# ubc-vision/UniT

Hardware: AMD Instinct MI355X
Metric: images/sec (fwd+bwd+SGD) R101-C4 VOC 600x1000 bs=2/GPU (higher is better)
Workload: dtype bf16; 1 GPU; UniT base-training step S1 (TrainerNoMeta.run_step): ResNet-101-C4, VOC split1 K=20, 2 supervised + 2 weak 3x600x1000 images per GPU, 512 RoIs/image, two Res5 heads, RPN 12000->2000, all 8 losses, SGD momentum; images_per_gpu=2, global_batch=2, parallelism=dp1

## Files before the change

### unit_amd/csrc/conv_igemm256.h

```cpp
#pragma once
#include "common.h"

#include "conv_epilogue.h"

struct Conv256Args {
  const void* x; const void* w; void* y;
  const float* bias; const void* residual; const void* mask_ref;
  int N, H, W, C;
  int K, R, S, stride, pad;
  int OH, OW;
  int ldy, oy_mul, OHf, OWf;
  int relu;
  int Kgemm, M;
  int tiles_m, tiles_n;
  unsigned x_bytes, w_bytes;
  EpiExtra ex;
  int ex_on;
  const void* x2; unsigned x2_bytes; int cb_split, ratio2;
  int pm_ncls;
  PmClass pm_cls[9];
  unsigned magic_ow, magic_oh;
  ConvSecond second;
  SplitK sk;
  int mask_pitch;
// ... 10 lines not shown
};
template <> struct O4<bf16_t> {
  static __device__ __forceinline__ void load(const bf16_t* p, float (&v)[4]) {
    bf16x4 a = *reinterpret_cast<const bf16x4*>(p);
#pragma unroll
    for (int i = 0; i < 4; ++i) v[i] = (float)a[i];
  }
  static __device__ __forceinline__ void store(bf16_t* p, const float (&v)[4]) {
    bf16x4 a;
#pragma unroll
    for (int i = 0; i < 4; ++i) a[i] = (bf16_t)v[i];
    *reinterpret_cast<bf16x4*>(p) = a;
  }
};

int unit_conv256_p8_launch(Conv256Args& a, int out_dtype, bool reads_in_mfma, bool rows224, hipStream_t st);
int unit_conv256_p8m_launch(Conv256Args& a, int out_dtype, hipStream_t st);
```

### unit_amd/csrc/conv_igemm256.hip

```cpp
#include "conv_igemm256.h"
#include "conv_igemm128.h"
#include "conv_pair.h"
#include "conv_epilogue.h"

#ifndef UNIT_DBG256
#define UNIT_DBG256 0
#endif

template <typename TO, bool PP, int FB>
__global__ void __launch_bounds__(512, 2) conv_igemm256_kernel(Conv256Args p) {
  constexpr int BM = 32 * FB, BMR = 256, BN = 256, BK = 64;
  constexpr int BUF = (BMR + BN) * 128;
  extern __shared__ __attribute__((aligned(16))) char smem[];

  int nwg = p.tiles_m * p.tiles_n;
  int bid = blockIdx.x;
  {
    int q = nwg / 8, r = nwg % 8, xcd = bid % 8, loc = bid / 8;
    bid = (xcd < r ? xcd * (q + 1) : r * (q + 1) + (xcd - r) * q) + loc;
  }
  int tile_n = bid % p.tiles_n, tile_m = bid / p.tiles_n;
  int m0 = tile_m * BM, n0 = tile_n * BN;

  const bf16_t* __restrict__ X = (const bf16_t*)p.x;
// ... 556 lines not shown
  a.sk = SplitK{0, 0, 0, 0}; a.mask_pitch = 0; a.second.on = 0;
  a.x = x; a.w = w; a.y = y; a.bias = bias; a.residual = residual; a.mask_ref = mask_ref;
  a.N = N; a.H = H; a.W = W; a.C = C; a.K = K; a.R = R; a.S = S; a.stride = stride; a.pad = pad;
  a.OH = OH; a.OW = OW; a.ldy = ldy; a.oy_mul = oy_mul; a.OHf = OHf; a.OWf = OWf; a.relu = relu;
  a.Kgemm = R * S * C; a.M = N * OH * OW;
  size_t xb = (size_t)N * H * W * C * 2, wb = (size_t)K * R * S * C * 2;
  UNIT_CHECK_ARG(xb < 0xFFFFFFF0ull && wb < 0xFFFFFFF0ull, "conv_big: operand larger than 4 GiB");
  a.x_bytes = (unsigned)xb; a.w_bytes = (unsigned)wb;
  a.ex = EpiExtra{nullptr, nullptr, nullptr, 0}; a.ex_on = 0;
  a.x2 = nullptr; a.x2_bytes = 0; a.cb_split = 0; a.ratio2 = 1; a.pm_ncls = 0;
  set_div_magics(a);
  { int rc = unit_fill_second(a.second, second, R, S, stride, pad, oy_mul, (size_t)C * 2); if (rc != UNIT_OK) return rc; }
  if (K == 0 || (a.M == 0 && !a.second.on)) return UNIT_OK;
  hipStream_t st = (hipStream_t)stream;
  if (variant == 0) variant = 8;
  if (a.second.on) {
    UNIT_CHECK_ARG(out_dtype == UNIT_BF16 && (ldy & 7) == 0 && (variant == 8 || variant == 12), "conv_big: pair launches: bf16 output, ldy % 8 == 0, variant 0 / 8 / 12");
    return unit_conv256_p8_launch(a, out_dtype, true, false, st);
  }
  auto fewer_with_224 = [&] {
    long n_tiles = cdiv(K, 256);
    long c256 = (long)cdiv((long)cdiv(a.M, 256) * n_tiles, 256) * 256, c224 = (long)cdiv((long)cdiv(a.M, 224) * n_tiles, 256) * 224;
    return c224 < c256;
  };
  if (variant == 6) {
    bool halo_ok = out_dtype == UNIT_BF16 && (ldy & 7) == 0 && R == 3 && S == 3 && stride == 1 && pad == 1 && H == 7 && W == 7 &&
                   OH == 7 && OW == 7;
    if (!halo_ok) { unit_set_error("conv_big: variant 6 needs a bf16-out 3x3 s1 p1 conv on 7x7 maps"); return UNIT_ERR_UNSUPPORTED; }
    return launch256_halo7(a, st);
  }
  if (variant == 11) return unit_conv256_p8m_launch(a, out_dtype, st);
  if (variant == 12) return unit_conv256_p8_launch(a, out_dtype, true, false, st);
  if (variant >= 7 && variant <= 10) {
    bool r224 = variant == 9 || (variant == 10 && fewer_with_224());
    if (variant == 8 && out_dtype == UNIT_BF16 && (ldy & 7) == 0 && R == 3 && S == 3 && stride == 1 &&
        pad == 1 && OH == H && OW == W && oy_mul == 1 && OHf == OH && OWf == OW && H * W <= 4096 && (size_t)N * H * W * ldy * 2 < 0xFFFFFFF0ull)
      build_position_classes(a);
    return unit_conv256_p8_launch(a, out_dtype, variant >= 8, r224, st);
  }
  bool rows224 = variant == 3 || (variant == 5 && fewer_with_224());
  if (out_dtype == UNIT_BF16) {
    if (variant == 2) return launch256_k32<bf16_t>(a, st);
    if (variant == 1) return launch256<bf16_t, true, 8>(a, st);
    return rows224 ? launch256<bf16_t, false, 7>(a, st) : launch256<bf16_t, false, 8>(a, st);
  }
  if (out_dtype == UNIT_F32) {
    if (variant == 2) return launch256_k32<float>(a, st);
    if (variant == 1) return launch256<float, true, 8>(a, st);
    return rows224 ? launch256<float, false, 7>(a, st) : launch256<float, false, 8>(a, st);
  }
  unit_set_error("conv_big: unsupported out dtype");
  return UNIT_ERR_UNSUPPORTED;
}
// ... 74 lines not shown
                                     second, stream, 3);
    case 4: return unit_conv_x3_impl(x, w, y, bias, residual, mask_ref, mask_c, N, H, W, C, K, R, S, stride, pad, OH, OW, ldy, oy_mul, OHf, OWf, relu, tile,
                                     second, stream, 2);
  }
  unit_set_error("conv_pair: kernel 0 (generic), 1 (mid), 2 (big), 3 (bf16x3), 4 (bf16x3, two segments)");
  return UNIT_ERR_ARG;
}


extern "C" size_t unit_conv_pool_partial_floats(int M, int ldy) { return (size_t)cdiv(M, 128) * 4 * (size_t)ldy; }

extern "C" int unit_conv2d_fwd_big_ex(const void* x, const void* w, void* y, const float* bias, const void* residual,
                                      const unsigned char* mask_bits, unsigned char* relu_bits, float* pool_partial, int pool_rows,
                                      int N, int H, int W, int C, int K, int R, int S, int pad, int ldy, int relu, const void* x2, int C2,
                                      int variant, void* stream) {
  UNIT_CHECK_ARG(variant == 0 || variant == 8 || variant == 11, "conv_big_ex: variant 0 (default), 8 (16x16x32 MFMA) or 11 (32x32x16 MFMA)");
  UNIT_CHECK_ARG(x2 == nullptr || (R == 1 && S == 1 && pad == 0 && C2 > 0 && C2 % C == 0 && ((uintptr_t)x2 % 16 == 0)),
                 "conv_big_ex: a second input needs a 1x1 conv and C2 a multiple of C");
  UNIT_CHECK_ARG(C % 64 == 0 && (x2 == nullptr || C2 % 64 == 0), "conv_big_ex: C must be a multiple of 64");
  UNIT_CHECK_ARG(ldy % 8 == 0 && ldy >= K, "conv_big_ex: ldy must be a multiple of 8 and >= K");
  UNIT_CHECK_ARG(y != nullptr || pool_partial != nullptr, "conv_big_ex: no output requested");
  UNIT_CHECK_ARG((mask_bits == nullptr && relu_bits == nullptr) || ldy % 64 == 0, "conv_big_ex: bit masks need ldy % 64 == 0");
  UNIT_CHECK_ARG(pool_partial == nullptr || pool_rows >= 44, "conv_big_ex: a 128-row wave tile must span at most 4 pooling segments");
  UNIT_CHECK_ARG(((uintptr_t)x % 16 == 0) && ((uintptr_t)w % 16 == 0) && ((uintptr_t)y % 16 == 0), "conv_big_ex: 16B alignment");
  int OH = H + 2 * pad - R + 1, OW = W + 2 * pad - S + 1;
  UNIT_CHECK_ARG(OH > 0 && OW > 0, "conv_big_ex: empty output");
  Conv256Args a;
  a.sk = SplitK{0, 0, 0, 0}; a.mask_pitch = 0; a.second.on = 0;
  a.x = x; a.w = w; a.y = y; a.bias = bias; a.residual = residual; a.mask_ref = nullptr;
  const int Ct = C + (x2 ? C2 : 0);
  a.N = N; a.H = H; a.W = W; a.C = Ct; a.K = K; a.R = R; a.S = S; a.stride = 1; a.pad = pad;
  a.OH = OH; a.OW = OW; a.ldy = ldy; a.oy_mul = 1; a.OHf = OH; a.OWf = OW; a.relu = relu;
  a.Kgemm = R * S * Ct; a.M = N * OH * OW;
  size_t xb = (size_t)N * H * W * C * 2, wb = (size_t)K * R * S * Ct * 2, x2b = x2 ? (size_t)N * H * W * C2 * 2 : 0;
  UNIT_CHECK_ARG(xb < 0xFFFFFFF0ull && wb < 0xFFFFFFF0ull && x2b < 0xFFFFFFF0ull, "conv_big_ex: operand larger than 4 GiB");
  a.x_bytes = (unsigned)xb; a.w_bytes = (unsigned)wb;
  a.x2 = x2; a.x2_bytes = (unsigned)x2b; a.cb_split = C / 64; a.ratio2 = x2 ? C2 / C : 1; a.pm_ncls = 0;
  set_div_magics(a);
  a.ex = EpiExtra{relu_bits, mask_bits, pool_partial, pool_rows}; a.ex_on = 1;
  if (a.M == 0 || K == 0) return UNIT_OK;
  if (variant == 11) return unit_conv256_p8m_launch(a, UNIT_BF16, (hipStream_t)stream);
  return unit_conv256_p8_launch(a, UNIT_BF16, true, false, (hipStream_t)stream);
}

template <typename T>
__global__ void pool_finish_kernel(const float* __restrict__ part, int R, int rows, int ldy, int K, T* __restrict__ out, int ldo) {
  int r = blockIdx.x;
  int w0 = (r * rows) / 128, w1 = (r * rows + rows - 1) / 128;
  float inv = (float)rows;
  int seg0 = r - (w0 * 128) / rows, seg1 = r - (w1 * 128) / rows;
  const float* p0 = part + ((size_t)w0 * 4 + seg0) * ldy;
  const float* p1 = part + ((size_t)w1 * 4 + seg1) * ldy;
  if ((K & 7) == 0 && (ldy & 3) == 0) {
    for (int n = threadIdx.x * 8; n < K; n += blockDim.x * 8) {
      f32x4 a0 = *reinterpret_cast<const f32x4*>(p0 + n), a1 = *reinterpret_cast<const f32x4*>(p0 + n + 4);
      f32x4 b0 = {0.f, 0.f, 0.f, 0.f}, b1 = {0.f, 0.f, 0.f, 0.f};
      if (w1 != w0) { b0 = *reinterpret_cast<const f32x4*>(p1 + n); b1 = *reinterpret_cast<const f32x4*>(p1 + n + 4); }
// ... 74 lines not shown
```

### unit_amd/csrc/conv_igemm256p8.hip

```cpp
#include "conv_igemm256.h"
#include "conv_epilogue.h"

#ifndef UNIT_DBGP8
#define UNIT_DBGP8 0
#endif

#ifdef UNIT_EPI_STAMP
__device__ unsigned long long g_stamp[32 * 16];
extern "C" int unit_debug_read_stamps(unsigned long long* host_out) {
  return (int)hipMemcpyFromSymbol(host_out, HIP_SYMBOL(g_stamp), sizeof(unsigned long long) * 32 * 16, 0, hipMemcpyDeviceToHost);
}
#define P8_STAMP(i) do { if (stamp) stamp[(i)] = __builtin_amdgcn_s_memtime(); } while (0)
#else
#define P8_STAMP(i) do { } while (0)
#endif

#define MFMA_BF16(A, B, C) __builtin_amdgcn_mfma_f32_16x16x32_bf16(__builtin_bit_cast(bf16x8, A), __builtin_bit_cast(bf16x8, B), C, 0, 0, 0)

template <typename TO, bool RM, int B1, bool X3 = false, bool PAIR = false, bool PERS = false>
__global__ void __launch_bounds__(512, 2) conv_igemm256_p8_kernel(Conv256Args p) {
  static_assert(RM || B1 == 4, "224-row tiles: RM schedule only");
  static_assert(!PAIR || (RM && B1 == 4), "pair launches: 256-row RM schedule");
  static_assert(!X3 || (RM && sizeof(TO) == 2), "bf16x3 operands: RM schedule, split bf16 output");
  static_assert(!PERS || (RM && !PAIR && sizeof(TO) == 2), "persistent tiles: RM schedule, bf16 rows through the LDS epilogue, one problem");
  constexpr int FBT = 4 + B1;
  constexpr int BM = 32 * FBT, BN = 256, BK = 64;
  constexpr int HALF = 128 * 128;
  constexpr int SX0 = 0, SW0 = HALF, SW1 = 2 * HALF, SX1 = 3 * HALF, BUF = 4 * HALF;
  constexpr int EPI_OFF = PERS ? BUF + SX1 : 0;
  extern __shared__ __attribute__((aligned(16))) char smem[];

  int bid = blockIdx.x;
  if constexpr (PAIR) {
    if (p.second.on && bid >= p.second.tiles0) { bid -= p.second.tiles0; pair_swap_common(p); p.magic_ow = p.second.magic_ow; p.magic_oh = p.second.magic_oh; }
  }
// ... 23 lines not shown
    int q = nwg / 8, r = nwg % 8, xcd = v % 8, loc = v / 8;
    int t = (xcd < r ? xcd * (q + 1) : r * (q + 1) + (xcd - r) * q) + loc;
    tile_n = t % p.tiles_n; tile_m = t / p.tiles_n;
  };
  if (!pm) map_tile(bid);
  int m0 = tile_m * BM, n0 = tile_n * BN;

  const bf16_t* __restrict__ X = (const bf16_t*)p.x;
  const bf16_t* __restrict__ Wt = (const bf16_t*)p.w;
  __amdgpu_buffer_rsrc_t rsX = __builtin_amdgcn_make_buffer_rsrc(const_cast<bf16_t*>(X), 0, (int)p.x_bytes, 0x00020000);
  __amdgpu_buffer_rsrc_t rsW = __builtin_amdgcn_make_buffer_rsrc(const_cast<bf16_t*>(Wt), 0, (int)p.w_bytes, 0x00020000);
  const bool dual = !X3 && p.x2 != nullptr;
  const int Cx = X3 ? p.sk.x_pitch : (dual ? p.cb_split * 64 : p.C);
  __amdgpu_buffer_rsrc_t rsX2 = __builtin_amdgcn_make_buffer_rsrc(const_cast<bf16_t*>((const bf16_t*)(dual ? p.x2 : p.x)), 0, (int)(dual ? p.x2_bytes : p.x_bytes), 0x00020000);
  constexpr unsigned OOB = 0xFFFFFFF0u;

  int tid = threadIdx.x, lane = tid & 63;
  int wid = __builtin_amdgcn_readfirstlane(tid >> 6);
  int wm = wid >> 2, wn = wid & 3;
  const int grp = wm;
  unsigned long long* stamp = nullptr;
#ifdef UNIT_EPI_STAMP
  if (tid == 0 && blockIdx.x % 97 == 0 && blockIdx.x / 97 < 32) {
    stamp = g_stamp + (blockIdx.x / 97) * 16;
    stamp[14] = blockIdx.x; stamp[15] = __builtin_amdgcn_s_memrealtime();
  }
#endif
  P8_STAMP(0);
  int lrow = lane >> 3, lc = lane & 7;

  const bool pointwise = PERS || (p.R == 1 && p.S == 1 && p.stride == 1 && p.pad == 0);
  int x_ih0[4], x_iw0[4]; unsigned x_off0[4], w_off[4];
  const unsigned sw16 = (unsigned)((lc ^ ((((wid * 8 + lrow) >> 1)) & 7)) * 16);
  auto setup_tile = [&](int lrow, int lc) {
#pragma unroll
  for (int q = 0; q < 2; ++q)
#pragma unroll
    for (int j = 0; j < 2; ++j) {
      int R = (j * 8 + wid) * 8 + lrow;
      int sw = lc ^ ((R >> 1) & 7);
      int m = m0 + (R >> 6) * (FBT * 16) + q * 64 + (R & 63);
      bool ok = m < p.M && (q == 0 || (R & 63) < B1 * 16);
      int mm = ok ? m : 0;
      int ow, oh, n;
      if (pm) {
        ok = pmr.map(m - m0, n, oh, ow);
        if (!ok) n = 0;
      } else if (pointwise) {
        n = 0; oh = 0; ow = 0;
      } else {
        unsigned t = fast_div((unsigned)mm, (unsigned)p.OW, p.magic_ow);
        ow = mm - (int)t * p.OW;
        n = (int)fast_div(t, (unsigned)p.OH, p.magic_oh);
        oh = (int)t - n * p.OH;
      }
      int ih0 = oh * p.stride - p.pad, iw0 = ow * p.stride - p.pad;
      x_off0[q * 2 + j] = pointwise ? ((unsigned)mm * (unsigned)Cx + (unsigned)(sw * 8)) * 2u
                                    : ((unsigned)n * (unsigned)(p.H * p.W * Cx) + (unsigned)((ih0 * p.W + iw0) * Cx + sw * 8)) * 2u;
      if constexpr (PERS) {
        if (!ok) x_off0[q * 2 + j] = OOB;
      } else {
        x_ih0[q * 2 + j] = ok ? ih0 : -(1 << 20);
        x_iw0[q * 2 + j] = iw0;
      }
      int nn = n0 + (R >> 5) * 64 + q * 32 + (R & 31);
      w_off[q * 2 + j] = nn < p.K ? ((unsigned)nn * (unsigned)p.Kgemm + (unsigned)sw * 8u) * 2u : OOB;
    }
  };
  setup_tile(lrow, lc);

  int r_lo = 0, r_hi = p.R - 1, s_lo = 0, s_hi = p.S - 1;
  if (pm) {
    r_lo = max(0, p.pad - pmr.oh0); r_hi = min(p.R - 1, p.H - 1 + p.pad - (pmr.oh0 + pm_nh - 1));
    s_lo = max(0, p.pad - pmr.ow0); s_hi = min(p.S - 1, p.W - 1 + p.pad - (pmr.ow0 + pmr.cw - 1));
  }
  int st_cb = 0, st_r = r_lo, st_s = s_lo;
  int st_sg = 0, st_cbr = 0;
  unsigned st_kx = (unsigned)((st_r * p.W + st_s) * Cx) * 2u, st_kw = (unsigned)((st_r * p.S + st_s) * p.C) * 2u;
  if constexpr (X3) st_kx += (unsigned)((p.sk.seg_lo & 1) * p.sk.cr) * 2u;
  auto st_reset = [&]() {
    st_cb = 0; st_r = r_lo; st_s = s_lo; st_sg = 0; st_cbr = 0;
// ... 36 lines not shown
      unsigned o = w_off[q * 2 + j];
      __builtin_amdgcn_raw_ptr_buffer_load_lds(rsW, (lds_void*)(base + (j * 8 + wid) * 1024), 16, o == OOB ? OOB : o + st_kw, 0, 0, 0);
    }
  };

  f32x4 acc[4][FBT];
  auto zero_acc = [&]() {
#pragma unroll
    for (int a = 0; a < 4; ++a)
#pragma unroll
      for (int b = 0; b < FBT; ++b) acc[a][b] = f32x4{0.f, 0.f, 0.f, 0.f};
  };
  zero_acc();

  const int nk = pm ? (p.C / BK) * (r_hi - r_lo + 1) * (s_hi - s_lo + 1) : p.Kgemm / BK;
  const int frow = lane & 15, fq = lane >> 4;
  const int fsw = (fq ^ ((frow >> 1) & 7)) << 4;
  const int offx = (wm * 64 + frow) * 128 + fsw;
  const int offw = (wn * 32 + frow) * 128 + fsw;

  i32x4 fx[4][2], fw0[2][2], fw1[2][2];
  auto read_x = [&](const char* half) {
#pragma unroll
    for (int b = 0; b < 4; ++b) {
      fx[b][0] = *reinterpret_cast<const i32x4*>(half + b * 2048 + offx);
      fx[b][1] = *reinterpret_cast<const i32x4*>(half + b * 2048 + (offx ^ 64));
    }
  };
  auto read_w = [&](const char* half, i32x4 (&fw)[2][2]) {
#pragma unroll
// ... 47 lines not shown
        }
      }
      if constexpr (RM && B1 == 4) {
        if (pm) {
          epilogue_rows_bf16_dispatch<4, FBT, false, true, false, EPI_BIAS | EPI_RELU | EPI_Y, EPI_MK | EPI_Y, EPI_Y>(
              acc, smem + EPI_OFF + wid * EpiCfg<4>::BYTES, nullptr, wm * (FBT * 16), n0e + wn * 64, p, lane, &pmr);
          return;
        }
      }
      epilogue_rows_bf16_dispatch<4, FBT, false, false, false, EPI_FULL | EPI_BIAS | EPI_RELU | EPI_Y, EPI_FULL | EPI_BIAS | EPI_Y, EPI_FULL | EPI_Y,
                                  EPI_FULL | EPI_MK | EPI_Y, EPI_FULL | EPI_RES | EPI_MK | EPI_Y, EPI_BIAS | EPI_RELU | EPI_Y, EPI_MK | EPI_Y>(
          acc, smem + EPI_OFF + wid * EpiCfg<4>::BYTES, nullptr, m0e + wm * (FBT * 16), n0e + wn * 64, p, lane, nullptr, stamp ? stamp + 4 : nullptr);
    }
  };

  if constexpr (RM) {
    constexpr int RD_PER = 1;
    i32x4 fxb[B1][2];
    auto read_xb = [&](const char* half) {
#pragma unroll
      for (int b = 0; b < B1; ++b) {
        fxb[b][0] = *reinterpret_cast<const i32x4*>(half + b * 2048 + offx);
        fxb[b][1] = *reinterpret_cast<const i32x4*>(half + b * 2048 + (offx ^ 64));
      }
    };
#define P8_MM(QX, QW, FW, FX, NB, NR, PER, READS)                                        \
    do {                                                                                 \
      __builtin_amdgcn_s_setprio(1);                                                     \
      READS;                                                                             \
      _Pragma("unroll") for (int ks = 0; ks < 2; ++ks)                                   \
        _Pragma("unroll") for (int a = 0; a < 2; ++a)                                    \
// ... 11 lines not shown
      stage_x(0, 0); stage_w(0, 0); stage_w(1, 0); stage_x(1, 0);
      st_advance();
      if (nk > 1) { stage_x(0, 1); stage_w(0, 1); stage_w(1, 1); }
    };
    prologue_stage();
    if (nk > 1) asm volatile("s_waitcnt vmcnt(6)" ::: "memory");
    else asm volatile("s_waitcnt vmcnt(0)" ::: "memory");
    int pers_v = blockIdx.x;
    while (true) {
    P8_BAR();
    P8_STAMP(1);
    read_w(smem + SW0, fw0);
    read_x(smem + SX0);
    asm volatile("s_waitcnt lgkmcnt(0)" ::: "memory");
    if (grp == 1) P8_BAR();
    for (int t = 0; t < nk; ++t) {
      const int d = t & 1;
      const char* buf = smem + d * BUF;
      const char* bnx = smem + (d ^ 1) * BUF;
      const bool n1 = t + 1 < nk, n2 = t + 2 < nk;
      if (n1) stage_x(1, d ^ 1);
      st_advance();
      P8_BAR();
      P8_MM(0, 0, fw0, fx, 4, 4, 1, read_w(buf + SW1, fw1));
      P8_BAR();
      if (n2) stage_x(0, d);
      P8_BAR();
      P8_MM(0, 1, fw1, fx, 4, 2 * B1, RD_PER, read_xb(buf + SX1));
      P8_BAR();
      if (n2) {
        stage_w(0, d);
        asm volatile("s_waitcnt vmcnt(4)" ::: "memory");
      } else {
        asm volatile("s_waitcnt vmcnt(0)" ::: "memory");
      }
      P8_BAR();
      P8_MM(1, 0, fw0, fxb, B1, 0, 1, (void)0);
      P8_BAR();
      if (n2) stage_w(1, d);
      P8_BAR();
      P8_MM(1, 1, fw1, fxb, B1, 12, RD_PER, read_w(bnx + SW0, fw0); read_x(bnx + SX0));
      P8_BAR();
    }
    if (grp == 0) P8_BAR();
    if constexpr (!PERS) break;
    else {
      P8_STAMP(2);
      __syncthreads();
      P8_STAMP(3);
      const int m0e = m0, n0e = n0, nv = pers_v + (int)gridDim.x;
      const bool more = nv < nwg;
      const bool early = more && !(p.ex_on && p.ex.pool_partial != nullptr);
      int lane_o = lane;
      asm volatile("" : "+v"(lane_o));
      auto next_tile = [&]() { map_tile(nv); m0 = tile_m * BM; n0 = tile_n * BN; setup_tile(lane_o >> 3, lane_o & 7); st_reset(); prologue_stage(); };
      if (early) next_tile();
      lds_epilogue(m0e, n0e, lane_o);
      if (!more) return;
      if (!early) { __syncthreads(); next_tile(); }
// ... 56 lines not shown
    P8_MFMA(1, 1, fw1);
    P8_BAR();
  }
  if (grp == 0) P8_BAR();
  }
#undef P8_MFMA
#undef P8_FMA
#undef P8_RD
#undef P8_BAR

  if constexpr (sizeof(TO) == 2) {
    if ((p.ldy & 7) == 0) {
      P8_STAMP(2);
      __syncthreads();
      P8_STAMP(3);
      lds_epilogue(m0, n0, lane);
      P8_STAMP(13);
      return;
    }
  }
  TO* __restrict__ Y = (TO*)p.y;
  const TO* __restrict__ Rz = (const TO*)p.residual;
  const TO* __restrict__ Mk = (const TO*)p.mask_ref;
  bool plain = (p.oy_mul == 1 && p.OHf == p.OH && p.OWf == p.OW);
#pragma unroll
  for (int b = 0; b < FBT; ++b) {
    int m = m0 + wm * (FBT * 16) + b * 16 + frow;
    if (m >= p.M) continue;
    long off;
    if (plain) off = (long)m * p.ldy;
// ... 17 lines not shown
      }
      if (p.relu) {
#pragma unroll
        for (int j = 0; j < 4; ++j) v[j] = fmaxf(v[j], 0.f);
      }
      if (Mk) {
        float mm[4]; O4<TO>::load(Mk + off + n, mm);
#pragma unroll
        for (int j = 0; j < 4; ++j) v[j] = mm[j] > 0.f ? v[j] : 0.f;
      }
      O4<TO>::store(Y + off + n, v);
    }
  }
}

template <typename TO, bool RM, int B1, bool X3 = false>
static int launch256_p8(Conv256Args& a, hipStream_t st) {
  if (a.second.on) {
    if constexpr (RM && B1 == 4 && sizeof(TO) == 2) {
      a.pm_ncls = 0;
      a.tiles_m = cdiv(a.M, 256); a.tiles_n = cdiv(a.K, 256);
      a.second.tiles_m = cdiv(a.second.M, 256);
      a.second.tiles0 = a.tiles_m * a.tiles_n;
      size_t lds2 = 8 * 128 * 128;
      static bool attr2 = false;
      if (!attr2) {
        (void)hipFuncSetAttribute((const void*)conv_igemm256_p8_kernel<TO, RM, B1, X3, true>, hipFuncAttributeMaxDynamicSharedMemorySize, (int)lds2);
        attr2 = true;
      }
      conv_igemm256_p8_kernel<TO, RM, B1, X3, true><<<(a.tiles_m + a.second.tiles_m) * a.tiles_n, 512, lds2, st>>>(a);
      UNIT_LAUNCH_CHECK();
      return UNIT_OK;
    } else {
      unit_set_error("conv_big: pair launches need the 256-row RM schedule with bf16 output");
      return UNIT_ERR_UNSUPPORTED;
    }
  }
  if (a.pm_ncls == 0) a.tiles_m = cdiv(a.M, 32 * (4 + B1));
  a.tiles_n = cdiv(a.K, 256);
  int grid = a.tiles_m * a.tiles_n;
  if (a.pm_ncls > 0) {
    if (!RM || B1 != 4) { unit_set_error("conv_big: position-class tiles need the 256-row RM schedule"); return UNIT_ERR_UNSUPPORTED; }
    int most = 0;
    for (int x = 0; x < 8; ++x) {
      int cnt = 0;
// ... 1 lines not shown
        int tc = (c + 1 < a.pm_ncls ? a.pm_cls[c + 1].tile0 : a.tiles_m) - a.pm_cls[c].tile0;
        cnt += ((x + 1) * tc + 7) / 8 - (x * tc + 7) / 8;
      }
      most = cnt > most ? cnt : most;
    }
    grid = most * 8 * a.tiles_n;
  }
  size_t lds = 8 * 128 * 128;
  if constexpr (RM && B1 == 4 && sizeof(TO) == 2) {
    const char* pe = getenv("UNIT_P8_PERSIST");
    const int pers = pe ? atoi(pe) : 1;
    if (pers && a.pm_ncls == 0 && (a.ldy & 7) == 0 && grid > 256 && a.R == 1 && a.S == 1 && a.stride == 1 && a.pad == 0) {
      const size_t lds_p = 7 * 128 * 128 + 8 * EpiCfg<4>::BYTES;
      static bool attr_p = false;
      if (!attr_p) {
        (void)hipFuncSetAttribute((const void*)conv_igemm256_p8_kernel<TO, RM, B1, X3, false, true>, hipFuncAttributeMaxDynamicSharedMemorySize, (int)lds_p);
        attr_p = true;
      }
      static int ncu = 0;
      if (ncu == 0) {
        int dev = 0, n = 0;
        if (hipGetDevice(&dev) != hipSuccess || hipDeviceGetAttribute(&n, hipDeviceAttributeMultiprocessorCount, dev) != hipSuccess || n < 8) n = 256;
        ncu = n / 8 * 8;
      }
      conv_igemm256_p8_kernel<TO, RM, B1, X3, false, true><<<grid < ncu ? grid : ncu, 512, lds_p, st>>>(a);
      UNIT_LAUNCH_CHECK();
      return UNIT_OK;
    }
  }
  static bool attr_set = false;
  if (!attr_set) {
    (void)hipFuncSetAttribute((const void*)conv_igemm256_p8_kernel<TO, RM, B1, X3>, hipFuncAttributeMaxDynamicSharedMemorySize, (int)lds);
    attr_set = true;
  }
  conv_igemm256_p8_kernel<TO, RM, B1, X3><<<grid, 512, lds, st>>>(a);
  UNIT_LAUNCH_CHECK();
  return UNIT_OK;
}

int unit_conv256_p8_launch(Conv256Args& a, int out_dtype, bool reads_in_mfma, bool rows224, hipStream_t st) {
  if (a.sk.nseg > 1) {
    if (out_dtype != UNIT_BF16 || (a.ldy & 7) != 0 || rows224 || !reads_in_mfma) { unit_set_error("conv_big: bf16x3 operands need the 256-row RM schedule and split output rows of 16-byte vectors"); return UNIT_ERR_UNSUPPORTED; }
    return launch256_p8<bf16_t, true, 4, true>(a, st);
  }
  if (rows224 && !reads_in_mfma) { unit_set_error("conv_big: 224-row tiles need the reads-in-MFMA schedule"); return UNIT_ERR_UNSUPPORTED; }
  if (out_dtype == UNIT_BF16) return rows224 ? launch256_p8<bf16_t, true, 3>(a, st) : reads_in_mfma ? launch256_p8<bf16_t, true, 4>(a, st) : launch256_p8<bf16_t, false, 4>(a, st);
  if (out_dtype == UNIT_F32) return rows224 ? launch256_p8<float, true, 3>(a, st) : reads_in_mfma ? launch256_p8<float, true, 4>(a, st) : launch256_p8<float, false, 4>(a, st);
  unit_set_error("conv_big: unsupported out dtype");
  return UNIT_ERR_UNSUPPORTED;
}
```

### unit_amd/ops.py

```python
import ctypes
import os
import math

import torch

from ._lib import _DEBUG_SYNC, check, lib

F32, BF16 = 0, 1
SCALE_CLAMP = math.log(1000.0 / 16)


def dt(dtype):
    if dtype == torch.float32:
        return F32
    if dtype == torch.bfloat16:
        return BF16
    raise TypeError(f"unsupported dtype {dtype}")


def _p(t):
    if t is None:
        return None
    if not t.is_cuda:
        raise RuntimeError("unit_amd ops need tensors on the ROCm device (no CPU fallback)")
# ... 192 lines not shown
    8: ("mid", 1),
    9: ("mid", 2),
    10: ("mid", 3),
    11: ("big", 2),
    12: ("big", 3),
    13: ("big", 4),
    14: ("big", 6),
    15: ("big", 7),
    16: ("big", 8),
    17: ("big", 9),
    18: ("big", 10),
    19: ("mid", 4),
    20: ("mid", 5),
    21: ("big", 11),
    22: ("big", 12),
}

WGRAD_STREAM = None
WGRAD_ACCUMULATE = False
WGRAD_DIRECT = False

PROFILER = None


class _timed:

    def __init__(self, name, flops=0.0, nbytes=0.0, ref_bytes=None):
        self.name, self.flops, self.nbytes, self.ref_bytes = name, flops, nbytes, ref_bytes

    def __enter__(self):
# ... 131 lines not shown
        else:
            out = torch.empty((n, ohf, owf, ldy), dtype=out_dtype, device=x.device)
    prof = PROFILER
    if prof is not None:
        e0 = torch.cuda.Event(enable_timing=True)
        e0.record()
    big, mid, variant = False, -1, 0
    if tile_cfg == 0:
        pkey = (x.dtype, n * oh * ow, k, c, r * s * c, out_dtype, ldy % 8, BIG_TILE_POLICY, MID_TILE_POLICY)
        pol = _POLICY_CACHE.get(pkey)
        if pol is None:
            pol = _POLICY_CACHE[pkey] = select_conv_kernel(x.dtype, n * oh * ow, k, c, r * s * c, out_dtype, ldy)
        big, mid = pol
    elif tile_cfg >= 100:
        mid = tile_cfg
    elif tile_cfg in TILE_CFG:
        kind, code = TILE_CFG[tile_cfg]
        if kind == "big":
            big, variant = True, code
        else:
            mid = code
    if mid >= 0:
        check(lib().unit_conv2d_fwd_mid(_p(x), _p(w), _p(out), _p(bias), _p(residual), _p(mask_ref), dt(out_dtype),
                                        n, h, wd, c, k, r, s, stride, pad, oh, ow, ldy, oy_mul, ohf, owf, int(relu), mid, _s()),
              "unit_conv2d_fwd_mid")
    elif big:
        check(lib().unit_conv2d_fwd_big(_p(x), _p(w), _p(out), _p(bias), _p(residual), _p(mask_ref), dt(out_dtype),
                                        n, h, wd, c, k, r, s, stride, pad, oh, ow, ldy, oy_mul, ohf, owf, int(relu),
                                        variant, _s()),
              "unit_conv2d_fwd_big")
    else:
        check(lib().unit_conv2d_fwd(_p(x), _p(w), _p(out), _p(bias), _p(residual), _p(mask_ref), dt(x.dtype), dt(out_dtype),
# ... 1077 lines not shown
```

Baseline: 139.0 images/sec.

## Add rewritten 256-row conv main loop with bitmask halo checks and ping-pong LDS pointers

Adds a new main-loop instantiation (LP=1) for the bf16 256-row reads-in-MFMA implicit-GEMM conv, used by default when the sizes fit. Padding checks become a precomputed per-row tap bitmask that ORs an out-of-range offset into the buffer load. Stepping over (r,s,cblock) is now branchless with uniform scalars, and the LDS read pointers ping-pong between buffers instead of being recomputed from the buffer index. The old loop stays reachable through variants 13/14. This adds complexity and limits which operand sizes can use the new path.

```diff
diff --git a/unit_amd/csrc/conv_igemm256.h b/unit_amd/csrc/conv_igemm256.h
--- a/unit_amd/csrc/conv_igemm256.h
+++ b/unit_amd/csrc/conv_igemm256.h
@@ -48,5 +48,5 @@
   }
 };
 
-int unit_conv256_p8_launch(Conv256Args& a, int out_dtype, bool reads_in_mfma, bool rows224, hipStream_t st);
+int unit_conv256_p8_launch(Conv256Args& a, int out_dtype, bool reads_in_mfma, bool rows224, hipStream_t st, int loop = 1);
 int unit_conv256_p8m_launch(Conv256Args& a, int out_dtype, hipStream_t st);
diff --git a/unit_amd/csrc/conv_igemm256.hip b/unit_amd/csrc/conv_igemm256.hip
--- a/unit_amd/csrc/conv_igemm256.hip
+++ b/unit_amd/csrc/conv_igemm256.hip
@@ -594,9 +594,11 @@
   if (K == 0 || (a.M == 0 && !a.second.on)) return UNIT_OK;
   hipStream_t st = (hipStream_t)stream;
   if (variant == 0) variant = 8;
+  int loop = 1;
+  if (variant == 13 || variant == 14) { loop = 0; variant = variant == 13 ? 8 : 12; }
   if (a.second.on) {
-    UNIT_CHECK_ARG(out_dtype == UNIT_BF16 && (ldy & 7) == 0 && (variant == 8 || variant == 12), "conv_big: pair launches: bf16 output, ldy % 8 == 0, variant 0 / 8 / 12");
-    return unit_conv256_p8_launch(a, out_dtype, true, false, st);
+    UNIT_CHECK_ARG(out_dtype == UNIT_BF16 && (ldy & 7) == 0 && (variant == 8 || variant == 12), "conv_big: pair launches: bf16 output, ldy % 8 == 0, variant 0 / 8 / 12 / 13 / 14");
+    return unit_conv256_p8_launch(a, out_dtype, true, false, st, loop);
   }
   auto fewer_with_224 = [&] {
     long n_tiles = cdiv(K, 256);
@@ -610,13 +612,13 @@
     return launch256_halo7(a, st);
   }
   if (variant == 11) return unit_conv256_p8m_launch(a, out_dtype, st);
-  if (variant == 12) return unit_conv256_p8_launch(a, out_dtype, true, false, st);
+  if (variant == 12) return unit_conv256_p8_launch(a, out_dtype, true, false, st, loop);
   if (variant >= 7 && variant <= 10) {
     bool r224 = variant == 9 || (variant == 10 && fewer_with_224());
     if (variant == 8 && out_dtype == UNIT_BF16 && (ldy & 7) == 0 && R == 3 && S == 3 && stride == 1 &&
         pad == 1 && OH == H && OW == W && oy_mul == 1 && OHf == OH && OWf == OW && H * W <= 4096 && (size_t)N * H * W * ldy * 2 < 0xFFFFFFF0ull)
       build_position_classes(a);
-    return unit_conv256_p8_launch(a, out_dtype, variant >= 8, r224, st);
+    return unit_conv256_p8_launch(a, out_dtype, variant >= 8, r224, st, loop);
   }
   bool rows224 = variant == 3 || (variant == 5 && fewer_with_224());
   if (out_dtype == UNIT_BF16) {
@@ -721,7 +723,8 @@
                                       const unsigned char* mask_bits, unsigned char* relu_bits, float* pool_partial, int pool_rows,
                                       int N, int H, int W, int C, int K, int R, int S, int pad, int ldy, int relu, const void* x2, int C2,
                                       int variant, void* stream) {
-  UNIT_CHECK_ARG(variant == 0 || variant == 8 || variant == 11, "conv_big_ex: variant 0 (default), 8 (16x16x32 MFMA) or 11 (32x32x16 MFMA)");
+  UNIT_CHECK_ARG(variant == 0 || variant == 8 || variant == 11 || variant == 13,
+                 "conv_big_ex: variant 0 (default), 8 (16x16x32 MFMA), 11 (32x32x16 MFMA) or 13 (8 on its loop of round 7)");
   UNIT_CHECK_ARG(x2 == nullptr || (R == 1 && S == 1 && pad == 0 && C2 > 0 && C2 % C == 0 && ((uintptr_t)x2 % 16 == 0)),
                  "conv_big_ex: a second input needs a 1x1 conv and C2 a multiple of C");
   UNIT_CHECK_ARG(C % 64 == 0 && (x2 == nullptr || C2 % 64 == 0), "conv_big_ex: C must be a multiple of 64");
@@ -747,7 +750,7 @@
   a.ex = EpiExtra{relu_bits, mask_bits, pool_partial, pool_rows}; a.ex_on = 1;
   if (a.M == 0 || K == 0) return UNIT_OK;
   if (variant == 11) return unit_conv256_p8m_launch(a, UNIT_BF16, (hipStream_t)stream);
-  return unit_conv256_p8_launch(a, UNIT_BF16, true, false, (hipStream_t)stream);
+  return unit_conv256_p8_launch(a, UNIT_BF16, true, false, (hipStream_t)stream, variant == 13 ? 0 : 1);
 }
 
 template <typename T>
diff --git a/unit_amd/csrc/conv_igemm256p8.hip b/unit_amd/csrc/conv_igemm256p8.hip
--- a/unit_amd/csrc/conv_igemm256p8.hip
+++ b/unit_amd/csrc/conv_igemm256p8.hip
@@ -15,10 +15,44 @@
 #define P8_STAMP(i) do { } while (0)
 #endif
 
+#ifdef UNIT_EPI_STAMP
+__device__ unsigned long long g_loop_stamp[64 * 16];
+extern "C" int unit_debug_read_loop_stamps(unsigned long long* host_out) {
+  return (int)hipMemcpyFromSymbol(host_out, HIP_SYMBOL(g_loop_stamp), sizeof(unsigned long long) * 64 * 16, 0, hipMemcpyDeviceToHost);
+}
+#define P8L_INIT()                                                                                        \
+  unsigned ts[12];                                                                                        \
+  _Pragma("unroll") for (int i = 0; i < 12; ++i) ts[i] = 0;                                               \
+  bool lstamp_on = (wid & 3) == 0 && blockIdx.x % 29 == 0 && blockIdx.x / 29 < 32;                        \
+  const int lstamp_t = nk >> 1;                                                                           \
+  if (lstamp_on) ts[11] = (unsigned)__builtin_amdgcn_s_memtime()
+#define P8L(i) do { if (lstamp_on) ts[(i)] = (unsigned)__builtin_amdgcn_s_memtime(); } while (0)
+#define P8L_T(i) do { if (lstamp_on && t == lstamp_t) ts[(i)] = (unsigned)__builtin_amdgcn_s_memtime(); } while (0)
+#define P8L_FLUSH()                                                                                       \
+  do {                                                                                                    \
+    if (lstamp_on && lane == 0) {                                                                         \
+      unsigned long long* g = g_loop_stamp + ((blockIdx.x / 29) * 2 + (wid >> 2)) * 16;                   \
+      _Pragma("unroll") for (int i = 0; i < 12; ++i) g[i] = ts[i];                                        \
+      g[13] = (unsigned long long)nk; g[14] = blockIdx.x; g[15] = (unsigned long long)wid;                \
+    }                                                                                                     \
+    lstamp_on = false;                                                                                    \
+  } while (0)
+#else
+#define P8L_INIT() do { } while (0)
+#define P8L(i) do { } while (0)
+#define P8L_T(i) do { } while (0)
+#define P8L_FLUSH() do { } while (0)
+#endif
+
+#ifndef UNIT_P8_RD_M2
+#define UNIT_P8_RD_M2 0
+#endif
+
 #define MFMA_BF16(A, B, C) __builtin_amdgcn_mfma_f32_16x16x32_bf16(__builtin_bit_cast(bf16x8, A), __builtin_bit_cast(bf16x8, B), C, 0, 0, 0)
 
-template <typename TO, bool RM, int B1, bool X3 = false, bool PAIR = false, bool PERS = false>
+template <typename TO, bool RM, int B1, bool X3 = false, bool PAIR = false, bool PERS = false, int LP = 0>
 __global__ void __launch_bounds__(512, 2) conv_igemm256_p8_kernel(Conv256Args p) {
+  static_assert(LP == 0 || (RM && B1 == 4 && !X3 && sizeof(TO) == 2), "new loop: bf16 256-row RM instantiations, plain operands");
   static_assert(RM || B1 == 4, "224-row tiles: RM schedule only");
   static_assert(!PAIR || (RM && B1 == 4), "pair launches: 256-row RM schedule");
   static_assert(!X3 || (RM && sizeof(TO) == 2), "bf16x3 operands: RM schedule, split bf16 output");
@@ -72,6 +106,7 @@
   const int Cx = X3 ? p.sk.x_pitch : (dual ? p.cb_split * 64 : p.C);
   __amdgpu_buffer_rsrc_t rsX2 = __builtin_amdgcn_make_buffer_rsrc(const_cast<bf16_t*>((const bf16_t*)(dual ? p.x2 : p.x)), 0, (int)(dual ? p.x2_bytes : p.x_bytes), 0x00020000);
   constexpr unsigned OOB = 0xFFFFFFF0u;
+  constexpr unsigned OOBX = 0xC0000000u;
 
   int tid = threadIdx.x, lane = tid & 63;
   int wid = __builtin_amdgcn_readfirstlane(tid >> 6);
@@ -89,7 +124,12 @@
 
   const bool pointwise = PERS || (p.R == 1 && p.S == 1 && p.stride == 1 && p.pad == 0);
   int x_ih0[4], x_iw0[4]; unsigned x_off0[4], w_off[4];
+  unsigned x_bad[4];
   const unsigned sw16 = (unsigned)((lc ^ ((((wid * 8 + lrow) >> 1)) & 7)) * 16);
+  auto bit_range = [](int lo, int hi) { return hi < lo ? 0u : ((2u << (hi - lo)) - 1u) << lo; };
+  unsigned tap_rep = 0;
+  if constexpr (LP == 1 && !PERS)
+    for (int r = 0; r < p.R; ++r) tap_rep |= 1u << (r * p.S);
   auto setup_tile = [&](int lrow, int lc) {
 #pragma unroll
   for (int q = 0; q < 2; ++q)
@@ -115,14 +155,19 @@
       int ih0 = oh * p.stride - p.pad, iw0 = ow * p.stride - p.pad;
       x_off0[q * 2 + j] = pointwise ? ((unsigned)mm * (unsigned)Cx + (unsigned)(sw * 8)) * 2u
                                     : ((unsigned)n * (unsigned)(p.H * p.W * Cx) + (unsigned)((ih0 * p.W + iw0) * Cx + sw * 8)) * 2u;
-      if constexpr (PERS) {
+      if constexpr (LP == 1 && PERS) {
+        if (!ok) x_off0[q * 2 + j] = OOBX;
+      } else if constexpr (LP == 1) {
+        const int rl = max(0, -ih0), rh = min(p.R - 1, p.H - 1 - ih0), sl = max(0, -iw0), sh = min(p.S - 1, p.W - 1 - iw0);
+        x_bad[q * 2 + j] = ok ? (~bit_range(rl * p.S, rh * p.S + p.S - 1) | (~bit_range(sl, sh) & bit_range(0, p.S - 1)) * tap_rep) : ~0u;
+      } else if constexpr (PERS) {
         if (!ok) x_off0[q * 2 + j] = OOB;
       } else {
         x_ih0[q * 2 + j] = ok ? ih0 : -(1 << 20);
         x_iw0[q * 2 + j] = iw0;
       }
       int nn = n0 + (R >> 5) * 64 + q * 32 + (R & 31);
-      w_off[q * 2 + j] = nn < p.K ? ((unsigned)nn * (unsigned)p.Kgemm + (unsigned)sw * 8u) * 2u : OOB;
+      w_off[q * 2 + j] = nn < p.K ? ((unsigned)nn * (unsigned)p.Kgemm + (unsigned)sw * 8u) * 2u : (LP == 1 ? OOBX : OOB);
     }
   };
   setup_tile(lrow, lc);
@@ -189,6 +234,7 @@
   zero_acc();
 
   const int nk = pm ? (p.C / BK) * (r_hi - r_lo + 1) * (s_hi - s_lo + 1) : p.Kgemm / BK;
+  P8L_INIT();
   const int frow = lane & 15, fq = lane >> 4;
   const int fsw = (fq ^ ((frow >> 1) & 7)) << 4;
   const int offx = (wm * 64 + frow) * 128 + fsw;
@@ -266,7 +312,177 @@
     }
   };
 
-  if constexpr (RM) {
+  if constexpr (RM && LP == 1) {
+    constexpr bool RD_M2 = UNIT_P8_RD_M2 != 0;
+    __amdgpu_buffer_rsrc_t rsXc = rsX;
+    auto uni = [](int v) { return __builtin_amdgcn_readfirstlane(v); };
+    s_lo = uni(s_lo); s_hi = uni(s_hi); r_lo = uni(r_lo); r_hi = uni(r_hi);
+    st_s = uni(st_s); st_r = uni(st_r); st_kx = (unsigned)uni((int)st_kx); st_kw = (unsigned)uni((int)st_kw);
+    const int ns = s_hi - s_lo, nr = r_hi - r_lo;
+    const unsigned kx_s = (unsigned)uni(Cx * 2), kx_r = (unsigned)uni((p.W - ns) * Cx * 2), kx_c = (unsigned)uni((BK - (nr * p.W + ns) * Cx) * 2);
+    const int tp_r = uni(p.S - ns), tp_c = uni(-(nr * p.S + ns)), kw_c = uni(p.C);
+    int st_tap = uni(st_r * p.S + st_s);
+    auto reset1 = [&]() { st_reset(); st_tap = st_r * p.S + st_s; rsXc = rsX; };
+    auto to_x2 = [&]() {
+      int l = lane;
+      asm volatile("" : "+v"(l));
+      const unsigned s16 = (unsigned)(((l & 7) ^ ((((wid * 8 + (l >> 3)) >> 1)) & 7)) * 16);
+#pragma unroll
+      for (int i = 0; i < 4; ++i) {
+        unsigned o2 = (x_off0[i] - s16) * (unsigned)p.ratio2;
+        asm volatile("" : "+v"(o2));
+        x_off0[i] = (PERS && x_off0[i] == OOBX) ? OOBX : o2 + s16;
+      }
+      rsXc = rsX2;
+    };
+    auto advance1 = [&]() {
+      bool wr = true;
+      if constexpr (PERS) {
+        ++st_cb; st_kx += BK * 2u; st_kw += BK * 2u;
+      } else {
+        const int ms = (s_hi - st_s - 1) >> 31;
+        const int mr = ms & ((r_hi - st_r - 1) >> 31);
+        wr = mr != 0;
+        st_s = (s_lo & ms) | ((st_s + 1) & ~ms);
+        st_r = (r_lo & mr) | ((st_r - ms) & ~mr);
+        st_cb -= mr;
+        st_kx += (kx_c & (unsigned)mr) | (kx_r & (unsigned)(ms & ~mr)) | (kx_s & (unsigned)~ms);
+        st_tap += (tp_c & mr) | (tp_r & ms & ~mr) | (1 & ~ms);
+        st_kw = (unsigned)(st_tap * kw_c + st_cb * BK) * 2u;
+      }
+      if (!PAIR && dual && wr && st_cb == p.cb_split) { to_x2(); st_kx = 0; }
+    };
+    auto stage_x1 = [&](int q, int d) {
+      char* base = smem + d * BUF + (q ? SX1 : SX0);
+#pragma unroll
+      for (int j = 0; j < 2; ++j) {
+        unsigned o = x_off0[q * 2 + j] + st_kx;
+        if constexpr (!PERS) o |= (unsigned)__builtin_amdgcn_sbfe((int)x_bad[q * 2 + j], (unsigned)st_tap, 1u);
+        __builtin_amdgcn_raw_ptr_buffer_load_lds(rsXc, (lds_void*)(base + (j * 8 + wid) * 1024), 16, o, 0, 0, 0);
+      }
+    };
+    auto stage_w1 = [&](int q, int d) {
+      char* base = smem + d * BUF + (q ? SW1 : SW0);
+#pragma unroll
+      for (int j = 0; j < 2; ++j)
+        __builtin_amdgcn_raw_ptr_buffer_load_lds(rsW, (lds_void*)(base + (j * 8 + wid) * 1024), 16, w_off[q * 2 + j] + st_kw, 0, 0, 0);
+    };
+    const char *bx0 = smem + offx, *bx1 = smem + (offx ^ 64), *bw0 = smem + offw, *bw1 = smem + (offw ^ 64);
+    int dfl = BUF;
+    auto flip = [&]() { bx0 += dfl; bx1 += dfl; bw0 += dfl; bw1 += dfl; dfl = -dfl; };
+    i32x4 fxb[4][2];
+    auto rd_x = [&](int slot, i32x4 (&f)[4][2]) {
+#pragma unroll
+      for (int b = 0; b < 4; ++b) {
+        f[b][0] = *reinterpret_cast<const i32x4*>(bx0 + slot + b * 2048);
+        f[b][1] = *reinterpret_cast<const i32x4*>(bx1 + slot + b * 2048);
+      }
+    };
+    auto rd_w = [&](int slot, i32x4 (&f)[2][2]) {
+#pragma unroll
+      for (int a = 0; a < 2; ++a) {
+        f[a][0] = *reinterpret_cast<const i32x4*>(bw0 + slot + a * 2048);
+        f[a][1] = *reinterpret_cast<const i32x4*>(bw1 + slot + a * 2048);
+      }
+    };
+#define P8_MM(QX, QW, FW, FX, NR, READS)                                                 \
+    do {                                                                                 \
+      __builtin_amdgcn_s_setprio(1);                                                     \
+      READS;                                                                             \
+      _Pragma("unroll") for (int ks = 0; ks < 2; ++ks)                                   \
+        _Pragma("unroll") for (int a = 0; a < 2; ++a)                                    \
+          _Pragma("unroll") for (int b = 0; b < 4; ++b)                                  \
+            acc[(QW) * 2 + a][(QX) * 4 + b] = MFMA_BF16(FW[a][ks], FX[b][ks], acc[(QW) * 2 + a][(QX) * 4 + b]); \
+      _Pragma("unroll") for (int i = 0; i < (NR); ++i) {                                 \
+        __builtin_amdgcn_sched_group_barrier(0x008, 1, 0);                               \
+        __builtin_amdgcn_sched_group_barrier(0x100, 1, 0);                               \
+      }                                                                                  \
+      __builtin_amdgcn_sched_group_barrier(0x008, 16 - (NR), 0);                         \
+      __builtin_amdgcn_s_setprio(0);                                                     \
+      if ((NR) > 0) asm volatile("s_waitcnt lgkmcnt(0)" ::: "memory");                   \
+    } while (0)
+    auto prologue_stage = [&]() {
+      stage_x1(0, 0); stage_w1(0, 0); stage_w1(1, 0); stage_x1(1, 0);
+      advance1();
+      if (nk > 1) { stage_x1(0, 1); stage_w1(0, 1); stage_w1(1, 1); }
+    };
+    prologue_stage();
+    if (nk > 1) asm volatile("s_waitcnt vmcnt(6)" ::: "memory");
+    else asm volatile("s_waitcnt vmcnt(0)" ::: "memory");
+    int pers_v = blockIdx.x;
+    while (true) {
+    P8_BAR();
+    P8_STAMP(1);
+    rd_w(SW0, fw0);
+    rd_x(SX0, fx);
+    asm volatile("s_waitcnt lgkmcnt(0)" ::: "memory");
+    if (grp == 1) P8_BAR();
+    P8L(9);
+    for (int t = 0; t < nk; ++t) {
+      const int d = t & 1;
+      const bool n1 = t + 1 < nk, n2 = t + 2 < nk;
+      P8L_T(0);
+      if (n1) stage_x1(1, d ^ 1);
+      advance1();
+      P8_BAR(); P8L_T(1);
+      P8_MM(0, 0, fw0, fx, 4, rd_w(SW1, fw1));
+      P8_BAR(); P8L_T(2);
+      if (n2) stage_x1(0, d);
+      if constexpr (RD_M2) {
+        if (n2) asm volatile("s_waitcnt vmcnt(8)" ::: "memory");
+        else if (n1) asm volatile("s_waitcnt vmcnt(6)" ::: "memory");
+      }
+      P8_BAR(); P8L_T(3);
+      P8_MM(0, 1, fw1, fx, 8, rd_x(SX1, fxb));
+      P8_BAR(); P8L_T(4);
+      if (n2) {
+        stage_w1(0, d);
+        asm volatile("s_waitcnt vmcnt(4)" ::: "memory");
+      } else {
+        asm volatile("s_waitcnt vmcnt(0)" ::: "memory");
+      }
+      flip();
+      P8_BAR(); P8L_T(5);
+      if constexpr (RD_M2) P8_MM(1, 0, fw0, fxb, 8, rd_x(SX0, fx));
+      else P8_MM(1, 0, fw0, fxb, 0, (void)0);
+      P8_BAR(); P8L_T(6);
+      if (n2) stage_w1(1, d);
+      P8_BAR(); P8L_T(7);
+      if constexpr (RD_M2) P8_MM(1, 1, fw1, fxb, 4, rd_w(SW0, fw0));
+      else P8_MM(1, 1, fw1, fxb, 12, rd_w(SW0, fw0); rd_x(SX0, fx));
+      P8_BAR(); P8L_T(8);
+    }
+    P8L(10);
+    if (grp == 0) P8_BAR();
+    P8L_FLUSH();
+    if (dfl < 0) flip();
+    if constexpr (!PERS) break;
+    else {
+      P8_STAMP(2);
+      __syncthreads();
+      P8_STAMP(3);
+      const int m0e = m0, n0e = n0, nv = pers_v + (int)gridDim.x;
+      const bool more = nv < nwg;
+      const bool early = more && !(p.ex_on && p.ex.pool_partial != nullptr);
+      int lane_o = lane;
+      asm volatile("" : "+v"(lane_o));
+      auto next_tile = [&]() { map_tile(nv); m0 = tile_m * BM; n0 = tile_n * BN; setup_tile(lane_o >> 3, lane_o & 7); reset1(); prologue_stage(); };
+      if (early) next_tile();
+      lds_epilogue(m0e, n0e, lane_o);
+      if (!more) return;
+      if (!early) { __syncthreads(); next_tile(); }
+      else {
+        asm volatile("" : "+s"(m0), "+s"(n0));
+        setup_tile(lane_o >> 3, lane_o & 7);
+        if (dual && st_cb >= p.cb_split) to_x2();
+      }
+      asm volatile("s_waitcnt vmcnt(0)" ::: "memory");
+      zero_acc();
+      pers_v = nv;
+    }
+    }
+#undef P8_MM
+  } else if constexpr (RM) {
     constexpr int RD_PER = 1;
     i32x4 fxb[B1][2];
     auto read_xb = [&](const char* half) {
@@ -308,35 +524,39 @@
     read_x(smem + SX0);
     asm volatile("s_waitcnt lgkmcnt(0)" ::: "memory");
     if (grp == 1) P8_BAR();
+    P8L(9);
     for (int t = 0; t < nk; ++t) {
       const int d = t & 1;
       const char* buf = smem + d * BUF;
       const char* bnx = smem + (d ^ 1) * BUF;
       const bool n1 = t + 1 < nk, n2 = t + 2 < nk;
+      P8L_T(0);
       if (n1) stage_x(1, d ^ 1);
       st_advance();
-      P8_BAR();
+      P8_BAR(); P8L_T(1);
       P8_MM(0, 0, fw0, fx, 4, 4, 1, read_w(buf + SW1, fw1));
-      P8_BAR();
+      P8_BAR(); P8L_T(2);
       if (n2) stage_x(0, d);
-      P8_BAR();
+      P8_BAR(); P8L_T(3);
       P8_MM(0, 1, fw1, fx, 4, 2 * B1, RD_PER, read_xb(buf + SX1));
-      P8_BAR();
+      P8_BAR(); P8L_T(4);
       if (n2) {
         stage_w(0, d);
         asm volatile("s_waitcnt vmcnt(4)" ::: "memory");
       } else {
         asm volatile("s_waitcnt vmcnt(0)" ::: "memory");
       }
-      P8_BAR();
+      P8_BAR(); P8L_T(5);
       P8_MM(1, 0, fw0, fxb, B1, 0, 1, (void)0);
-      P8_BAR();
+      P8_BAR(); P8L_T(6);
       if (n2) stage_w(1, d);
-      P8_BAR();
+      P8_BAR(); P8L_T(7);
       P8_MM(1, 1, fw1, fxb, B1, 12, RD_PER, read_w(bnx + SW0, fw0); read_x(bnx + SX0));
-      P8_BAR();
-    }
+      P8_BAR(); P8L_T(8);
+    }
+    P8L(10);
     if (grp == 0) P8_BAR();
+    P8L_FLUSH();
     if constexpr (!PERS) break;
     else {
       P8_STAMP(2);
@@ -423,6 +643,12 @@
       P8_STAMP(2);
       __syncthreads();
       P8_STAMP(3);
+      if constexpr (LP == 1) {
+        int lane_o = lane;
+        asm volatile("" : "+v"(lane_o));
+        lds_epilogue(m0, n0, lane_o);
+        return;
+      }
       lds_epilogue(m0, n0, lane);
       P8_STAMP(13);
       return;
@@ -470,7 +696,7 @@
   }
 }
 
-template <typename TO, bool RM, int B1, bool X3 = false>
+template <typename TO, bool RM, int B1, bool X3 = false, int LP = 0>
 static int launch256_p8(Conv256Args& a, hipStream_t st) {
   if (a.second.on) {
     if constexpr (RM && B1 == 4 && sizeof(TO) == 2) {
@@ -481,10 +707,10 @@
       size_t lds2 = 8 * 128 * 128;
       static bool attr2 = false;
       if (!attr2) {
-        (void)hipFuncSetAttribute((const void*)conv_igemm256_p8_kernel<TO, RM, B1, X3, true>, hipFuncAttributeMaxDynamicSharedMemorySize, (int)lds2);
+        (void)hipFuncSetAttribute((const void*)conv_igemm256_p8_kernel<TO, RM, B1, X3, true, false, LP>, hipFuncAttributeMaxDynamicSharedMemorySize, (int)lds2);
         attr2 = true;
       }
-      conv_igemm256_p8_kernel<TO, RM, B1, X3, true><<<(a.tiles_m + a.second.tiles_m) * a.tiles_n, 512, lds2, st>>>(a);
+      conv_igemm256_p8_kernel<TO, RM, B1, X3, true, false, LP><<<(a.tiles_m + a.second.tiles_m) * a.tiles_n, 512, lds2, st>>>(a);
       UNIT_LAUNCH_CHECK();
       return UNIT_OK;
     } else {
@@ -516,7 +742,7 @@
       const size_t lds_p = 7 * 128 * 128 + 8 * EpiCfg<4>::BYTES;
       static bool attr_p = false;
       if (!attr_p) {
-        (void)hipFuncSetAttribute((const void*)conv_igemm256_p8_kernel<TO, RM, B1, X3, false, true>, hipFuncAttributeMaxDynamicSharedMemorySize, (int)lds_p);
+        (void)hipFuncSetAttribute((const void*)conv_igemm256_p8_kernel<TO, RM, B1, X3, false, true, LP>, hipFuncAttributeMaxDynamicSharedMemorySize, (int)lds_p);
         attr_p = true;
       }
       static int ncu = 0;
@@ -525,27 +751,34 @@
         if (hipGetDevice(&dev) != hipSuccess || hipDeviceGetAttribute(&n, hipDeviceAttributeMultiprocessorCount, dev) != hipSuccess || n < 8) n = 256;
         ncu = n / 8 * 8;
       }
-      conv_igemm256_p8_kernel<TO, RM, B1, X3, false, true><<<grid < ncu ? grid : ncu, 512, lds_p, st>>>(a);
+      conv_igemm256_p8_kernel<TO, RM, B1, X3, false, true, LP><<<grid < ncu ? grid : ncu, 512, lds_p, st>>>(a);
       UNIT_LAUNCH_CHECK();
       return UNIT_OK;
     }
   }
   static bool attr_set = false;
   if (!attr_set) {
-    (void)hipFuncSetAttribute((const void*)conv_igemm256_p8_kernel<TO, RM, B1, X3>, hipFuncAttributeMaxDynamicSharedMemorySize, (int)lds);
+    (void)hipFuncSetAttribute((const void*)conv_igemm256_p8_kernel<TO, RM, B1, X3, false, false, LP>, hipFuncAttributeMaxDynamicSharedMemorySize, (int)lds);
     attr_set = true;
   }
-  conv_igemm256_p8_kernel<TO, RM, B1, X3><<<grid, 512, lds, st>>>(a);
+  conv_igemm256_p8_kernel<TO, RM, B1, X3, false, false, LP><<<grid, 512, lds, st>>>(a);
   UNIT_LAUNCH_CHECK();
   return UNIT_OK;
 }
 
-int unit_conv256_p8_launch(Conv256Args& a, int out_dtype, bool reads_in_mfma, bool rows224, hipStream_t st) {
+static bool new_loop_fits(const Conv256Args& a) {
+  const unsigned lim = 0xC0000000u;
+  return a.x_bytes <= lim && a.w_bytes <= lim && a.x2_bytes <= lim && (!a.second.on || a.second.x_bytes <= lim) && a.R * a.S <= 32 &&
+         (size_t)a.Kgemm * 2 < 0x3FFFFFF0ull && (size_t)(a.R * a.W + a.S) * (size_t)a.C * 2 < 0x3FFFFFF0ull;
+}
+
+int unit_conv256_p8_launch(Conv256Args& a, int out_dtype, bool reads_in_mfma, bool rows224, hipStream_t st, int loop) {
   if (a.sk.nseg > 1) {
     if (out_dtype != UNIT_BF16 || (a.ldy & 7) != 0 || rows224 || !reads_in_mfma) { unit_set_error("conv_big: bf16x3 operands need the 256-row RM schedule and split output rows of 16-byte vectors"); return UNIT_ERR_UNSUPPORTED; }
     return launch256_p8<bf16_t, true, 4, true>(a, st);
   }
   if (rows224 && !reads_in_mfma) { unit_set_error("conv_big: 224-row tiles need the reads-in-MFMA schedule"); return UNIT_ERR_UNSUPPORTED; }
+  if (out_dtype == UNIT_BF16 && reads_in_mfma && !rows224 && loop == 1 && new_loop_fits(a)) return launch256_p8<bf16_t, true, 4, false, 1>(a, st);
   if (out_dtype == UNIT_BF16) return rows224 ? launch256_p8<bf16_t, true, 3>(a, st) : reads_in_mfma ? launch256_p8<bf16_t, true, 4>(a, st) : launch256_p8<bf16_t, false, 4>(a, st);
   if (out_dtype == UNIT_F32) return rows224 ? launch256_p8<float, true, 3>(a, st) : reads_in_mfma ? launch256_p8<float, true, 4>(a, st) : launch256_p8<float, false, 4>(a, st);
   unit_set_error("conv_big: unsupported out dtype");
diff --git a/unit_amd/ops.py b/unit_amd/ops.py
--- a/unit_amd/ops.py
+++ b/unit_amd/ops.py
@@ -230,6 +230,10 @@
     20: ("mid", 5),
     21: ("big", 11),
     22: ("big", 12),
+}
+TILE_CFG_LOOP = {
+    23: ("big", 13),
+    24: ("big", 14),
 }
 
 WGRAD_STREAM = None
@@ -391,8 +395,8 @@
         big, mid = pol
     elif tile_cfg >= 100:
         mid = tile_cfg
-    elif tile_cfg in TILE_CFG:
-        kind, code = TILE_CFG[tile_cfg]
+    elif tile_cfg in TILE_CFG or tile_cfg in TILE_CFG_LOOP:
+        kind, code = TILE_CFG.get(tile_cfg) or TILE_CFG_LOOP[tile_cfg]
         if kind == "big":
             big, variant = True, code
         else:
```

Measured after the change: 140.3 images/sec, median of 6. About the same (+1.0%).
